# shionhonda/gae-dgl

Hardware: AMD Instinct MI355X
Metric: edges aggregated/sec (SpMM fwd+bwd) (higher is better)
Workload: dtype f32 (storage, aggregations, accumulators; the dense products run on the 16-bit matrix pipe from split operands with fp32 accumulation: X W^T and dW from three bf16 pieces per operand / six pairs, the loss from two fp16 pieces (N >= 5120) or three bf16 pieces -- all fp32-grade, see ms_per_step_exact_

## Files before the change

gae_dgl_amd/csrc/decoder_bce.hip:

```cpp
#include <string.h>

#include "common.h"
#include "bce_finalize.h"

namespace {

using gae::kWave;
typedef float f32x4 __attribute__((ext_vector_type(4)));
typedef short s16x4 __attribute__((ext_vector_type(4)));
typedef float f32x2 __attribute__((ext_vector_type(2)));
typedef __bf16 bf16x2 __attribute__((ext_vector_type(2)));

constexpr int TJ = 64;
constexpr int PREP_ROWS = 64;
constexpr int kBceRi = 2;
constexpr int64_t kBceGrid = 2048;
constexpr int64_t kBceSymGrid = 16384;
constexpr int kChipCus = 256;
}

namespace gae {
Knob g_bce_s_bf16{3};
Knob g_bce_last_kind{0};
Knob g_bce_sym_bal{1};
// ... 499 lines not shown
    }
#pragma unroll
    for (int off = 32; off > 0; off >>= 1) { la += __shfl_down(la, off, 64); ll += __shfl_down(ll, off, 64); }
    if (lane == 0) { red[wave][0] = la; red[wave][1] = ll; }
    __syncthreads();
    if (tid == 0) {
        const int64_t b = int64_t(blockIdx.y) * n_row_blocks + blockIdx.x;
        loss_partial[2 * b + 0] = (red[0][0] + red[1][0]) + (red[2][0] + red[3][0]);
        loss_partial[2 * b + 1] = (red[0][1] + red[1][1]) + (red[2][1] + red[3][1]);
    }
}

}

namespace gae {
Knob g_bce_sym_ri{0};
}

namespace {
using gae::g_bce_sym_ri;

__device__ __forceinline__ s16x4 upper_halves(const f32x4 &d)
{
    struct U { unsigned a, b; } u{__builtin_amdgcn_perm(__float_as_uint(d[1]), __float_as_uint(d[0]), 0x07060302u),
                                  __builtin_amdgcn_perm(__float_as_uint(d[3]), __float_as_uint(d[2]), 0x07060302u)};
    return __builtin_bit_cast(s16x4, u);
}

__host__ __device__ inline int64_t sym_strip_offset(int64_t I, int64_t NP, int64_t PR)
{
    return 16 * (I * NP - PR * (I * (I + 1) / 2));
}

enum class SymForm { kF16, kBf16x3, kBf16x3Fallback };

template <bool WITH_GRAD, int RI, SymForm FORM, bool BAL>
__global__ __launch_bounds__(256, (RI == 2 && FORM != SymForm::kBf16x3Fallback) ? 3 : 2) void bce_dense_sym_kernel(
    const float *__restrict__ Zt , const unsigned short *__restrict__ Zhi,
    const unsigned short *__restrict__ Zlo, int64_t n, int64_t cols_per_chunk,
    float *__restrict__ O_partial , float *__restrict__ Wmir,
    double *__restrict__ loss_partial , const double *__restrict__ colsum_partial,
    int64_t n_prep_blocks, double *__restrict__ S, float *__restrict__ S_all_f, unsigned n_panels, int exp_strip,
    unsigned *__restrict__ range_flag, int flag_mode, unsigned ticket, unsigned n_chunks, int bal_tpb)
{
    if (flag_mode == 2 && *range_flag != ticket) return;
    constexpr bool F16 = FORM == SymForm::kF16;
    constexpr bool PERSIST = FORM == SymForm::kBf16x3Fallback;
    bool out_of_range = false;
    constexpr int DP = 16, SYM_PR = 64 * RI;
    constexpr int LDH = DP + 4;
    constexpr int V4 = TJ * DP / 4 / 256;
    constexpr int LDM = TJ + 4;
    constexpr int LDHL = 2 * DP + 8;
    __shared__ __attribute__((aligned(16))) unsigned short HLs[2][TJ * LDHL];
    __shared__ __attribute__((aligned(16))) unsigned short L2s[2][F16 ? 4 : TJ * LDH];
    __shared__ __attribute__((aligned(16))) float MR[2][4][16 * LDM];
    __shared__ double red[4][2];

  double sumA = 0.0, sumL = 0.0;
  auto unit = [&](const int64_t I, const int64_t col_begin, const int64_t col_end, const int64_t op_slot, const int64_t lp_index) {
    const int tid = threadIdx.x, lane = tid & 63, wave = tid >> 6;
    const int l15 = lane & 15, g = lane >> 4;
    const int64_t NP = (n + 63) / 64 * 64;
    const int64_t row_base = SYM_PR * I + wave * (RI * 16);
    const int64_t diag_end = SYM_PR * (I + 1);

    constexpr float LOG2E = 1.44269504088896341f;
    static_assert(RI % 2 == 0, "row subtiles are paired into K = 32 mirror products");
    s16x8 bhh[RI];
    s16x8 bll[RI];
    s16x8 b3[F16 ? 1 : RI];
    s16x8 zTh[RI / 2], zTl[RI / 2];
#pragma unroll
    for (int ri = 0; ri < RI; ++ri) {
        const int64_t i = row_base + ri * 16 + l15;
        f32x4 b = *reinterpret_cast<const f32x4 *>(Zt + (i < n ? i : 0) * DP + 4 * g);
// ... 254 lines not shown
            if (I > T - 1) I = T - 1;
            I = __builtin_amdgcn_readfirstlane(I);
            while (I > 0 && prefix(I) > t0) --I;
            while (I + 1 < T && prefix(I + 1) <= t0) ++I;
            while (t0 < t1) {
                const int pI = prefix(I), tiles = NT - TPP * I;
                const int lt = t0 - pI;
                int cnt = tiles - lt;
                if (cnt > t1 - t0) cnt = t1 - t0;
                const int64_t cb = int64_t(SYM_PR) * I + int64_t(lt) * 64;
                int64_t ce = cb + int64_t(cnt) * 64;
                if (ce > n) ce = n;
                if (cb < n) unit(I, cb, ce, int(vb) - int(unsigned(pI) / unsigned(bal_tpb)), -1);
                __syncthreads();
                t0 += cnt; ++I;
            }
        }
        const int tid = threadIdx.x, lane = tid & 63, wave = tid >> 6;
        double la = sumA * 0.69314718055994531, ll = sumL;
#pragma unroll
        for (int off = 32; off > 0; off >>= 1) { la += __shfl_down(la, off, 64); ll += __shfl_down(ll, off, 64); }
        if (lane == 0) { red[wave][0] = la; red[wave][1] = ll; }
        __syncthreads();
        if (tid == 0) {
            loss_partial[2 * vb + 0] = (red[0][0] + red[1][0]) + (red[2][0] + red[3][0]);
            loss_partial[2 * vb + 1] = (red[0][1] + red[1][1]) + (red[2][1] + red[3][1]);
        }
        };
        if constexpr (PERSIST) {
            for (unsigned vb = blockIdx.x; vb < n_vb; vb += gridDim.x) {
                vblock(vb);
                __syncthreads();
            }
        } else {
            vblock(blockIdx.x);
        }
    } else if constexpr (PERSIST) {
        const unsigned nx = n_panels + 1, total = nx * n_chunks;
        for (unsigned u = blockIdx.x; u < total; u += gridDim.x) {
            unit_xy(u % nx, u / nx);
            __syncthreads();
        }
    } else {
        unit_xy(blockIdx.x, blockIdx.y);
    }
}

__global__ __launch_bounds__(256) void bce_mirror_reduce_kernel(const float *__restrict__ Wmir, int64_t n,
                                                               float *__restrict__ Omir , int SYM_PR)
{
    const int64_t NP = (n + 63) / 64 * 64;
    const int64_t j0 = int64_t(blockIdx.x) * TJ;
    const int f = threadIdx.x >> 4, jq = (threadIdx.x & 15) * 4;
    const int64_t n_left = j0 / SYM_PR;
    f32x4 acc = {0.f, 0.f, 0.f, 0.f};
    auto at = [&](int64_t I) {
        const int64_t de = SYM_PR * (I + 1);
        return *reinterpret_cast<const f32x4 *>(Wmir + sym_strip_offset(I, NP, SYM_PR) + (j0 - de) * 16 + f * TJ + jq);
    };
    int64_t I = 0;
    for (; I + 8 <= n_left; I += 8) {
        f32x4 v[8];
#pragma unroll
        for (int u = 0; u < 8; ++u) v[u] = at(I + u);
#pragma unroll
        for (int u = 0; u < 8; ++u) acc += v[u];
    }
    for (; I < n_left; ++I) acc += at(I);
#pragma unroll
    for (int e = 0; e < 4; ++e)
        if (j0 + jq + e < n) Omir[(j0 + jq + e) * 16 + f] = acc[e];
}

template <int LPR, bool WITH_GRAD>
__global__ __launch_bounds__(256) void bce_edges_kernel(
    const float *__restrict__ Zt , const float *__restrict__ mask, int64_t ldz,
    int64_t row_begin, int64_t n_local, int d, const int32_t *__restrict__ indptr,
    const int32_t *__restrict__ indices, const int32_t *__restrict__ t_indptr, const int32_t *__restrict__ t_indices,
    float pw, float inv_n2, const float *__restrict__ O_partial, int n_splits, int DP,
    const float *__restrict__ S_all_f, float *__restrict__ dZ, int64_t lddz, double *__restrict__ loss_partial,
    const float *__restrict__ O_mirror , int64_t sym_cols_per_chunk, int SYM_PR,
    const int64_t *__restrict__ counts, const double *__restrict__ scal,
    const float *__restrict__ Wmir ,
    unsigned *__restrict__ range_flag )
{
    constexpr int VEC = 4;
    if (range_flag != nullptr && blockIdx.x == 0 && threadIdx.x == 0) *range_flag = 0u;
    const unsigned bid = (LPR == 4 && Wmir != nullptr) ? gridDim.x - 1u - blockIdx.x : blockIdx.x;
    __shared__ __attribute__((aligned(16))) float Om[LPR == 4 ? TJ * 20 : 4];
    const bool fold = LPR == 4 && Wmir != nullptr;
    if (LPR == 4 && fold) {
        const int64_t NP = (n_local + 63) / 64 * 64;
        const int64_t j0 = int64_t(bid) * TJ;
        const int f = threadIdx.x >> 4, jq = (threadIdx.x & 15) * 4;
        const int64_t n_left = j0 / SYM_PR;
        f32x4 acc = {0.f, 0.f, 0.f, 0.f};
        auto at = [&](int64_t I) {
            const int64_t de = SYM_PR * (I + 1);
            return *reinterpret_cast<const f32x4 *>(Wmir + sym_strip_offset(I, NP, SYM_PR) + (j0 - de) * 16 + f * TJ + jq);
        };
        int64_t I = 0;
        for (; I + 8 <= n_left; I += 8) {
            f32x4 v[8];
#pragma unroll
            for (int u = 0; u < 8; ++u) v[u] = at(I + u);
#pragma unroll
            for (int u = 0; u < 8; ++u) acc += v[u];
        }
        for (; I < n_left; ++I) acc += at(I);
#pragma unroll
        for (int e = 0; e < 4; ++e) Om[(jq + e) * 20 + f] = acc[e];
        __syncthreads();
    }
    if (scal) { pw = float(scal[0]); inv_n2 = float(scal[1]); }
    const int64_t n_valid = counts ? counts[0] : n_local;
    __shared__ double red[4];
    constexpr int RPB = 256 / LPR;
    const int tid = threadIdx.x, lane = tid & 63, wave = tid >> 6;
    const int lig = tid % LPR;
    const int64_t i = int64_t(bid) * RPB + tid / LPR;
    const int64_t gi = row_begin + i;
    const int64_t n = n_local;
    const int f0 = lig * VEC;
    const bool rowv = i < n;
    const bool fv = f0 < DP;

    float zi[VEC], acc_in[VEC], acc_out[VEC];
    const f32x4 zero4 = {0.f, 0.f, 0.f, 0.f};
    {
        const f32x4 t = (rowv && fv) ? *reinterpret_cast<const f32x4 *>(Zt + gi * DP + f0) : zero4;
#pragma unroll
        for (int q = 0; q < VEC; ++q) { acc_in[q] = acc_out[q] = 0.f; zi[q] = t[q]; }
    }
    float sall[VEC], mk[VEC];
#pragma unroll
    for (int q = 0; q < VEC; ++q) {
        const bool in = WITH_GRAD && rowv && f0 + q < d;
        sall[q] = WITH_GRAD ? S_all_f[in ? f0 + q : 0] : 0.f;
        mk[q] = (WITH_GRAD && mask != nullptr) ? mask[in ? gi * ldz + f0 + q : 0] : 1.f;
    }
    int32_t posA = rowv ? indptr[i] : 0;
    int32_t endA = rowv ? indptr[i + 1] : 0;
    int32_t posB = (WITH_GRAD && rowv) ? t_indptr[i] : 0;
    int32_t endB = (WITH_GRAD && rowv) ? t_indptr[i + 1] : 0;
    constexpr int kLongRow = 16;
    const bool is_long = max(endA - posA, endB - posB) > kLongRow;
    const int32_t longA0 = posA, longA1 = endA, longB0 = posB, longB1 = endB;
    if (is_long) { endA = posA; endB = posB; }
    f32x4 osum = zero4;
    if (WITH_GRAD && rowv && fv) {
        const float *op = O_partial + i * DP + f0;
        const int64_t sstride = n * DP;
        if (O_mirror) {
            if (sym_cols_per_chunk < 0) {
                const int64_t tpb = -sym_cols_per_chunk, I = i / SYM_PR, TPP = SYM_PR / 64, NT = (n + 63) / 64;
                const int64_t pI = I * NT - TPP * (I * (I - 1) / 2), pI1 = pI + NT - TPP * I;
                n_splits = int((pI1 - 1) / tpb - pI / tpb + 1);
            } else {
                const int64_t rem = n - (i / SYM_PR) * SYM_PR;
                n_splits = int((rem + sym_cols_per_chunk - 1) / sym_cols_per_chunk);
            }
            osum = fold ? *reinterpret_cast<const f32x4 *>(&Om[(tid / LPR) * 20 + f0])
                        : *reinterpret_cast<const f32x4 *>(O_mirror + i * DP + f0);
        }
        int sp = 0;
        for (; sp + 8 <= n_splits; sp += 8) {
            f32x4 o[8];
#pragma unroll
            for (int u = 0; u < 8; ++u) o[u] = *reinterpret_cast<const f32x4 *>(op + (sp + u) * sstride);
#pragma unroll
            for (int u = 0; u < 8; ++u) osum += o[u];
        }
        if (sp < n_splits) {
            f32x4 o[8];
#pragma unroll
            for (int u = 0; u < 8; ++u) {
                const int su = sp + u < n_splits ? sp + u : n_splits - 1;
                o[u] = *reinterpret_cast<const f32x4 *>(op + su * sstride);
            }
#pragma unroll
            for (int u = 0; u < 8; ++u) osum += (sp + u < n_splits) ? o[u] : zero4;
        }
    }
    double lsum = 0.0;
    constexpr int NE = LPR >= 4 ? 8 : 4;
    const int glane0 = (lane / LPR) * LPR;
    while (posA < endA || posB < endB) {
        int32_t mineA[NE / 4], mineB[NE / 4];
#pragma unroll
        for (int h = 0; h < NE / 4; ++h) {
            const int32_t eA = posA + 4 * h + (LPR >= 4 ? (lig & 3) : 0), eB = posB + 4 * h + (LPR >= 4 ? (lig & 3) : 0);
            mineA[h] = eA < endA ? indices[eA] : 0;
            mineB[h] = (WITH_GRAD && eB < endB) ? t_indices[eB] : 0;
        }
        float zj[2 * NE][VEC], dot[2 * NE];
#pragma unroll
        for (int u = 0; u < 2 * NE; ++u) {
            const bool second = u >= NE;
            if (second && !WITH_GRAD) { dot[u] = 0.f; continue; }
            const int32_t pos = second ? posB : posA, end = second ? endB : endA;
            const int uu = u % NE;
            const int32_t mine = second ? mineB[uu / 4] : mineA[uu / 4];
            const int32_t j = LPR >= 4 ? __shfl(mine, glane0 + (uu & 3), 64)
                                       : (pos + uu < end ? (second ? t_indices : indices)[pos + uu] : 0);
            const bool ev = pos + uu < end;
            dot[u] = 0.f;
            const f32x4 t = (ev && fv) ? *reinterpret_cast<const f32x4 *>(Zt + int64_t(j) * DP + f0) : zero4;
#pragma unroll
            for (int q = 0; q < VEC; ++q) {
                zj[u][q] = t[q];
                dot[u] = fmaf(zi[q], t[q], dot[u]);
            }
        }
#pragma unroll
        for (int off = LPR / 2; off > 0; off >>= 1)
#pragma unroll
            for (int u = 0; u < (WITH_GRAD ? 2 * NE : NE); ++u) dot[u] += __shfl_xor(dot[u], off, 64);
#pragma unroll
        for (int u = 0; u < (WITH_GRAD ? 2 * NE : NE); ++u) {
            const bool second = u >= NE;
            const int32_t pos = second ? posB : posA, end = second ? endB : endA;
            if (pos + (u % NE) < end) {
                const float x = dot[u];
                float spn, sgn;
                softplus_sigmoid(-x, spn, sgn);
                const float sg = 1.0f - sgn;
                if (!second && lig == 0) lsum += double(-x + (pw - 1.0f) * spn);
                const float c = (pw - 1.0f) * sg - pw;
#pragma unroll
                for (int q = 0; q < VEC; ++q) {
                    if (second) acc_out[q] = fmaf(c, zj[u][q], acc_out[q]);
                    else acc_in[q] = fmaf(c, zj[u][q], acc_in[q]);
                }
            }
        }
        posA = min(posA + NE, endA);
        posB = min(posB + NE, endB);
    }
    {
        constexpr int G = 64 / LPR, CU = LPR < 4 ? LPR : 4, CH = CU * G;
        unsigned long long todo = __builtin_amdgcn_ballot_w64(is_long && lig == 0);
        const int grp = lane / LPR;
        while (todo != 0) {
            const int hl = __builtin_ctzll(todo);
            todo &= todo - 1;
            const int32_t eA = __builtin_amdgcn_readlane(longA1, hl), eB = __builtin_amdgcn_readlane(longB1, hl);
            int32_t a0 = __builtin_amdgcn_readlane(longA0, hl), b0 = __builtin_amdgcn_readlane(longB0, hl);
            float zr[VEC], pin[VEC], pout[VEC];
#pragma unroll
            for (int q = 0; q < VEC; ++q) {
                zr[q] = __shfl(zi[q], hl + lig, 64);
                pin[q] = pout[q] = 0.f;
            }
            for (; a0 < eA || b0 < eB; a0 += CH, b0 += CH) {
                const int32_t idA = (lane < CH && a0 + lane < eA) ? indices[a0 + lane] : 0;
                const int32_t idB = (WITH_GRAD && lane < CH && b0 + lane < eB) ? t_indices[b0 + lane] : 0;
                float zj[2 * CU][VEC], dot[2 * CU];
#pragma unroll
                for (int u = 0; u < 2 * CU; ++u) {
                    const bool second = u >= CU;
                    dot[u] = 0.f;
                    if (second && !WITH_GRAD) continue;
                    const int slot = grp + G * (u % CU);
                    const int32_t j = __shfl(second ? idB : idA, slot, 64);
                    const bool ev = (second ? b0 : a0) + slot < (second ? eB : eA);
                    const f32x4 t = (ev && fv) ? *reinterpret_cast<const f32x4 *>(Zt + int64_t(j) * DP + f0) : zero4;
#pragma unroll
                    for (int q = 0; q < VEC; ++q) {
                        zj[u][q] = t[q];
                        dot[u] = fmaf(zr[q], t[q], dot[u]);
                    }
                }
#pragma unroll
                for (int off = LPR / 2; off > 0; off >>= 1)
#pragma unroll
                    for (int u = 0; u < (WITH_GRAD ? 2 * CU : CU); ++u) dot[u] += __shfl_xor(dot[u], off, 64);
#pragma unroll
                for (int u = 0; u < (WITH_GRAD ? 2 * CU : CU); ++u) {
                    const bool second = u >= CU;
                    const int slot = grp + G * (u % CU);
                    if ((second ? b0 : a0) + slot < (second ? eB : eA)) {
                        const float x = dot[u];
                        float spn, sgn;
                        softplus_sigmoid(-x, spn, sgn);
                        const float sg = 1.0f - sgn;
                        if (!second && lig == 0) lsum += double(-x + (pw - 1.0f) * spn);
                        const float c = (pw - 1.0f) * sg - pw;
#pragma unroll
                        for (int q = 0; q < VEC; ++q) {
                            if (second) pout[q] = fmaf(c, zj[u][q], pout[q]);
                            else pin[q] = fmaf(c, zj[u][q], pin[q]);
                        }
                    }
                }
            }
#pragma unroll
            for (int off = LPR; off < 64; off <<= 1)
#pragma unroll
                for (int q = 0; q < VEC; ++q) {
                    pin[q] += __shfl_xor(pin[q], off, 64);
                    if (WITH_GRAD) pout[q] += __shfl_xor(pout[q], off, 64);
                }
            if ((lane & ~(LPR - 1)) == hl) {
#pragma unroll
                for (int q = 0; q < VEC; ++q) { acc_in[q] += pin[q]; acc_out[q] += pout[q]; }
            }
        }
    }
    if (WITH_GRAD && rowv) {
#pragma unroll
        for (int q = 0; q < VEC; ++q) {
            const int f = f0 + q;
            if (f < d) {
                const float o = 0.5f * sall[q] + osum[q];
                float v = (2.0f * o + (acc_in[q] + acc_out[q])) * inv_n2;
                if (mask) v *= mk[q];
                if (i >= n_valid) v = 0.f;
                dZ[i * lddz + f] = v;
            }
        }
    }
#pragma unroll
    for (int off = 32; off > 0; off >>= 1) lsum += __shfl_down(lsum, off, 64);
    if (lane == 0) red[wave] = lsum;
    __syncthreads();
    if (tid == 0) loss_partial[bid] = (red[0] + red[1]) + (red[2] + red[3]);
}

__global__ __launch_bounds__(1024) void bce_finalize_kernel(const gae_bce_tail t)
{
    __shared__ double red[3][16];
    gae::bce_finalize_block<1024>(t, red);
}

struct BcePlan {
    int64_t row_blocks, n_splits, cols_per_split, edge_blocks, prep_blocks;
    int KS, DP, LPR;
    int64_t o_bytes, zt_bytes, zh_bytes, cs_bytes, s_bytes, n_dense, total_bytes;
    double pad_terms;
    bool sym;
    int sym_pr;
    int bal_tpb;
    int64_t bal_blocks;
    int64_t wmir_bytes, omir_bytes;
};

inline int64_t align256(int64_t x) { return (x + 255) / 256 * 256; }

bool bce_plan(int64_t n, int64_t n_local, int64_t d, BcePlan &p)
{
    const int64_t ROWS_PER_BLOCK = 64 * kBceRi;
    if (d > 64) return false;
    p.KS = int((d + 15) / 16);
    if (p.KS == 3) p.KS = 4;
    if (p.KS < 1) p.KS = 1;
    p.DP = p.KS * 16;
    p.row_blocks = (n_local + ROWS_PER_BLOCK - 1) / ROWS_PER_BLOCK;
    if (p.row_blocks < 1) p.row_blocks = 1;
    int64_t col_tiles = (n + TJ - 1) / TJ;
    if (col_tiles < 1) col_tiles = 1;
    int64_t want = (kBceGrid + p.row_blocks - 1) / p.row_blocks;
    if (want > col_tiles) want = col_tiles;
    if (want > 32) want = 32;
    if (want < 1) want = 1;
    const int64_t tiles_per_split = (col_tiles + want - 1) / want;
    p.cols_per_split = tiles_per_split * TJ;
    p.n_splits = (col_tiles + tiles_per_split - 1) / tiles_per_split;
    p.pad_terms = double(col_tiles * TJ - n) * double(n_local);
    const int nvec = p.DP / 4;
    int lpr = 1;
    while (lpr < nvec) lpr <<= 1;
    p.LPR = lpr;
    p.edge_blocks = (n_local + (256 / lpr) - 1) / (256 / lpr);
    if (p.edge_blocks < 1) p.edge_blocks = 1;
    p.prep_blocks = (n + PREP_ROWS - 1) / PREP_ROWS;
    p.sym = false;
    p.sym_pr = 128;
    p.bal_tpb = 0;
    p.bal_blocks = 0;
    p.wmir_bytes = p.omir_bytes = 0;
    const bool bal = g_bce_sym_bal == 2 || (g_bce_sym_bal == 1 && n < 65536);
    if (g_bce_sym && n_local == n && p.KS == 1 && g_bce_s_bf16 && g_bce_pv_bf16 &&
        n >= (g_bce_sym > 1 ? 512 : (bal ? 5120 : 8192))) {
        const int64_t SYM_PR = (g_bce_sym_ri == 4 || (g_bce_sym_ri == 0 && (n >= 32768 || bal))) ? 256 : 128;
        p.sym_pr = int(SYM_PR);
        const int64_t T = (n + SYM_PR - 1) / SYM_PR, NP = (n + 63) / 64 * 64;
        int64_t chunks = (kBceSymGrid + T - 1) / T;
        if (chunks > 28) chunks = 28;
        if (chunks > col_tiles) chunks = col_tiles;
        if (chunks < 1) chunks = 1;
        int64_t cpc = ((n + chunks - 1) / chunks + TJ - 1) / TJ * TJ;
        const int64_t slots = int64_t(kChipCus) * (SYM_PR == 128 ? 3 : 2);
        auto live_blocks = [&](int64_t t) {
            int64_t L = 0;
            for (int64_t I = 0; I < T; ++I) L += (n - SYM_PR * I + t * TJ - 1) / (t * TJ);
            return L;
        };
        const int64_t t0 = cpc / TJ;
        if ((live_blocks(t0) + slots - 1) / slots <= 6) {
            double best = -1.0;
            int64_t best_t = t0;
            for (int64_t t = t0 - t0 / 4; t <= t0 + t0 / 4; ++t) {
                if (t < 1) continue;
                const int64_t L = live_blocks(t), rounds = (L + slots - 1) / slots;
                const double fill = double(L) / double(rounds * slots) - 0.002 * double(t > t0 ? t - t0 : t0 - t);
                if (fill > best) { best = fill; best_t = t; }
            }
            cpc = best_t * TJ;
        }
        const int64_t last_len = NP - SYM_PR * T;
        const int64_t wfloats = sym_strip_offset(T - 1, NP, SYM_PR) + 16 * (last_len > 0 ? last_len : 0);
        if (wfloats * 4 <= (int64_t(8) << 30)) {
            p.sym = true;
            p.row_blocks = T;
            p.cols_per_split = cpc;
            p.n_splits = (n + cpc - 1) / cpc;
            p.pad_terms = 0.0;
            p.wmir_bytes = align256(wfloats * 4);
            p.omir_bytes = align256(n * 16 * 4);
            if (bal) {
                const int64_t TPP = SYM_PR / TJ, NT = NP / TJ;
                auto prefix = [&](int64_t I) { return I * NT - TPP * (I * (I - 1) / 2); };
                const int64_t W = prefix(T), slots = int64_t(kChipCus) * (SYM_PR == 128 ? 3 : 2);
                const int64_t tpb = (W + slots - 1) / slots;
                int64_t most = 1;
                for (int64_t I = 0; I < T; ++I) {
                    const int64_t pieces = (prefix(I + 1) - 1) / tpb - prefix(I) / tpb + 1;
                    if (pieces > most) most = pieces;
                }
                p.bal_tpb = int(tpb);
                p.bal_blocks = (W + tpb - 1) / tpb;
                p.n_splits = most;
            }
        }
    }
    p.o_bytes = align256(p.n_splits * n_local * p.DP * 4);
    p.zt_bytes = align256(n * p.DP * 4);
    p.zh_bytes = align256(n * p.DP * 2);
    p.cs_bytes = align256(((n + 15) / 16 + 1) * 2 * p.DP * 8);
    p.s_bytes = align256(2 * p.DP * 8 + p.DP * 4 + 4 * 8);
    p.n_dense = p.bal_tpb ? p.bal_blocks : p.row_blocks * p.n_splits;
    p.total_bytes = p.o_bytes + p.zt_bytes + 2 * p.zh_bytes + p.cs_bytes + p.s_bytes +
                    align256((2 * p.n_dense + p.edge_blocks) * 8) + p.wmir_bytes + p.omir_bytes;
    return true;
}

template <int KS, bool WITH_GRAD>
auto dense_kernel()
{
    if (!g_bce_s_bf16) return bce_dense_kernel<KS, WITH_GRAD, false, false>;
    return g_bce_pv_bf16 ? bce_dense_kernel<KS, WITH_GRAD, true, true> : bce_dense_kernel<KS, WITH_GRAD, true, false>;
}

template <bool WITH_GRAD>
int launch_dense(const BcePlan &p, const float *Zt, const unsigned short *Zhi, const unsigned short *Zlo, int64_t n,
                 int64_t row_begin, int64_t n_local, float *O, double *lp, const double *cs, double *S, float *S_all_f,
                 hipStream_t s)
{
    const dim3 grid(unsigned(p.row_blocks) + 1, unsigned(p.n_splits));
    const auto kernel = p.KS == 1 ? dense_kernel<1, WITH_GRAD>() : p.KS == 2 ? dense_kernel<2, WITH_GRAD>()
                                                                             : dense_kernel<4, WITH_GRAD>();
    hipLaunchKernelGGL(kernel, grid, dim3(256), 0, s, Zt, Zhi, Zlo, n, row_begin, n_local, p.cols_per_split, O, lp, cs,
                       p.prep_blocks, S, S_all_f, unsigned(p.row_blocks));
    GAE_CHECK_LAUNCH("bce_dense_kernel");
    return GAE_OK;
}

template <bool WITH_GRAD>
int launch_edges(const BcePlan &p, const float *Zt, const float *mask, int64_t ldz, int64_t row_begin, int64_t n, int d,
                 const int32_t *ip, const int32_t *ix, const int32_t *tp, const int32_t *tx, float pw, float inv_n2,
                 const float *O, const float *S_all_f, float *dZ, int64_t lddz, double *lp, const float *Omir,
                 const int64_t *counts, const double *scal, const float *Wmir, unsigned *range_flag, hipStream_t s)
{
    const auto kernel = p.LPR == 1 ? bce_edges_kernel<1, WITH_GRAD>
                        : p.LPR == 2 ? bce_edges_kernel<2, WITH_GRAD>
                        : p.LPR == 4 ? bce_edges_kernel<4, WITH_GRAD>
                        : p.LPR == 8 ? bce_edges_kernel<8, WITH_GRAD>
                                     : bce_edges_kernel<16, WITH_GRAD>;
    hipLaunchKernelGGL(kernel, dim3(unsigned(p.edge_blocks)), dim3(256), 0, s, Zt, mask, ldz, row_begin, n, d, ip, ix, tp,
                       tx, pw, inv_n2, O, int(p.n_splits), p.DP, S_all_f, dZ, lddz, lp, Omir,
                       (p.bal_tpb ? -int64_t(p.bal_tpb) : p.cols_per_split), p.sym_pr, counts, scal, Wmir, range_flag);
    GAE_CHECK_LAUNCH("bce_edges_kernel");
    return GAE_OK;
}

template <SymForm FORM>
auto sym_kernel(const BcePlan &p, bool with_grad)
{
    const bool tall = p.sym_pr == 256, bal = p.bal_tpb != 0;
    if (with_grad) {
        if (tall) return bal ? bce_dense_sym_kernel<true, 4, FORM, true> : bce_dense_sym_kernel<true, 4, FORM, false>;
        return bal ? bce_dense_sym_kernel<true, 2, FORM, true> : bce_dense_sym_kernel<true, 2, FORM, false>;
    }
    if (tall) return bal ? bce_dense_sym_kernel<false, 4, FORM, true> : bce_dense_sym_kernel<false, 4, FORM, false>;
    return bal ? bce_dense_sym_kernel<false, 2, FORM, true> : bce_dense_sym_kernel<false, 2, FORM, false>;
}

}

extern "C" int64_t gae_decoder_bce_workspace_bytes(int64_t n, int64_t n_local, int64_t d)
{
    if (n < 0 || d < 0 || n_local < 0 || n_local > n) return GAE_E_SIZE;
    BcePlan p;
    if (!bce_plan(n, n_local, d, p)) return GAE_E_RANGE;
    return p.total_bytes + 256;
}

namespace {
inline double bce_all_pairs(const BcePlan &p, int64_t n, int64_t n_local)
{
    return p.sym ? double(n) * double(n) : double(n_local) * double((n + TJ - 1) / TJ * TJ);
}

thread_local gae_bce_tail *t_tail_out = nullptr;
// ... 12 lines not shown
    GAE_REQUIRE(n > 0 && d > 0, GAE_E_SIZE, "gae_decoder_bce: n and d must be positive");
    GAE_REQUIRE(row_begin >= 0 && n_local >= 0 && row_begin + n_local <= n, GAE_E_SIZE,
                "gae_decoder_bce: row window outside [0, n)");
    GAE_REQUIRE(d <= 64, GAE_E_RANGE, "gae_decoder_bce: d = %lld > 64 not supported by the fused kernel",
                (long long)d);
    GAE_REQUIRE(n < (int64_t(1) << 31), GAE_E_SIZE, "gae_decoder_bce: n too large");
    GAE_REQUIRE(ldz >= d && (!dZ || lddz >= d), GAE_E_SIZE, "gae_decoder_bce: leading dimension too small");
    GAE_REQUIRE((Z || prepared) && loss_out && workspace && (n_local == 0 || indptr), GAE_E_NULL, "gae_decoder_bce: NULL pointer");
    GAE_REQUIRE(!dZ || n_local == 0 || t_indptr, GAE_E_NULL, "gae_decoder_bce: the gradient needs the CSR of A^T");
    BcePlan p;
    bce_plan(n, n_local, d, p);
    GAE_REQUIRE(workspace_bytes >= p.total_bytes, GAE_E_WORKSPACE, "gae_decoder_bce: workspace %lld < %lld bytes",
                (long long)workspace_bytes, (long long)p.total_bytes);
    if (prepared) {
        GAE_REQUIRE(prepared_blocks >= 1 && prepared_blocks * 2 * p.DP * 8 <= p.cs_bytes, GAE_E_RANGE,
                    "gae_x_decoder_bce_prepared: %lld column-sum partials do not fit the workspace", (long long)prepared_blocks);
        p.prep_blocks = prepared_blocks;
    }
    GAE_REQUIRE(gae::aligned16(workspace), GAE_E_ALIGN, "gae_decoder_bce: workspace not 16-byte aligned");
    hipStream_t s = gae::as_stream(stream);
    char *w = static_cast<char *>(workspace);
    float *O = reinterpret_cast<float *>(w); w += p.o_bytes;
    float *Zt = reinterpret_cast<float *>(w); w += p.zt_bytes;
    unsigned short *Zhi = reinterpret_cast<unsigned short *>(w); w += p.zh_bytes;
    unsigned short *Zlo = reinterpret_cast<unsigned short *>(w); w += p.zh_bytes;
    double *cs = reinterpret_cast<double *>(w); w += p.cs_bytes;
    double *S = reinterpret_cast<double *>(w);
    float *S_all_f = reinterpret_cast<float *>(w + 2 * p.DP * 8);
    double *scal = counts ? reinterpret_cast<double *>(w + 2 * p.DP * 8 + ((p.DP * 4 + 7) & ~7)) : nullptr;
    unsigned *range_flag = reinterpret_cast<unsigned *>(w + 2 * p.DP * 8 + ((p.DP * 4 + 7) & ~7) + 3 * 8);
    w += p.s_bytes;
    double *lp = reinterpret_cast<double *>(w); w += align256((2 * p.n_dense + p.edge_blocks) * 8);
    float *Wmir = reinterpret_cast<float *>(w); w += p.wmir_bytes;
    float *Omir = reinterpret_cast<float *>(w);
    const double inv_n2 = 1.0 / (double(n) * double(n));
    if (n_local == 0) {
        GAE_HIP(hipMemsetAsync(loss_out, 0, sizeof(float), s));
        if (t_tail_out) { memset(t_tail_out, 0, sizeof(gae_bce_tail)); t_tail_out = nullptr; }
        return GAE_OK;
    }
    if (!prepared) {
        hipLaunchKernelGGL(bce_prepare_kernel, dim3(unsigned(p.prep_blocks)), dim3(256), 0, s, Z, mask, ldz, n, int(d), p.DP,
                           row_begin, row_begin + n_local, Zt, Zhi, Zlo, cs, dropout_p, 1.0f / (1.0f - dropout_p), seed,
                           offset, draw_dev, counts, scal, bce_all_pairs(p, n, n_local));
        GAE_CHECK_LAUNCH("bce_prepare_kernel");
    }
    int rc;
    g_bce_last_kind = p.sym ? (p.sym_pr == 256 ? 3 : 2) : 1;
    if (p.sym) {
        const dim3 grid = p.bal_tpb ? dim3(unsigned(p.bal_blocks) + 1) : dim3(unsigned(p.row_blocks) + 1, unsigned(p.n_splits));
        static std::atomic<unsigned> call_counter{0};
        const unsigned ticket = (call_counter.fetch_add(1) * 2654435761u) | 0x80000001u;
        auto launch_sym = [&](auto kernel, dim3 g, int flag_mode) {
            hipLaunchKernelGGL(kernel, g, dim3(256), 0, s, Zt, Zhi, Zlo, n, p.cols_per_split, O, Wmir, lp, cs, p.prep_blocks, S,
                               S_all_f, unsigned(p.row_blocks), n >= 32768 ? 1 : 0, range_flag, flag_mode, ticket,
                               (p.bal_tpb ? unsigned(p.bal_blocks) + 1u : unsigned(p.n_splits)), p.bal_tpb);
        };
        if (g_bce_s_bf16 == 3) {
            launch_sym(sym_kernel<SymForm::kF16>(p, dZ != nullptr), grid, 1);
            launch_sym(sym_kernel<SymForm::kBf16x3Fallback>(p, dZ != nullptr), p.bal_tpb ? dim3(64) : dim3(2 * kChipCus), 2);
        } else {
            launch_sym(sym_kernel<SymForm::kBf16x3>(p, dZ != nullptr), grid, 0);
        }
        GAE_CHECK_LAUNCH("bce_dense_sym_kernel");
        if (dZ && p.LPR != 4) {
            hipLaunchKernelGGL(bce_mirror_reduce_kernel, dim3(unsigned((n + TJ - 1) / TJ)), dim3(256), 0, s, Wmir, n,
                               Omir, p.sym_pr);
            GAE_CHECK_LAUNCH("bce_mirror_reduce_kernel");
        }
        rc = GAE_OK;
    } else {
        rc = dZ ? launch_dense<true>(p, Zt, Zhi, Zlo, n, row_begin, n_local, O, lp, cs, S, S_all_f, s)
                : launch_dense<false>(p, Zt, Zhi, Zlo, n, row_begin, n_local, O, lp, cs, S, S_all_f, s);
    }
    if (rc) return rc;
    double *lpe = lp + 2 * p.n_dense;
    rc = dZ ? launch_edges<true>(p, Zt, mask, ldz, row_begin, n_local, int(d), indptr, indices, t_indptr, t_indices,
                                    pos_weight, float(inv_n2), O, S_all_f, dZ, lddz, lpe, p.sym ? Omir : nullptr,
                                    counts, scal, (p.sym && p.LPR == 4) ? Wmir : nullptr,
                                    p.sym ? range_flag : nullptr, s)
            : launch_edges<false>(p, Zt, mask, ldz, row_begin, n_local, int(d), indptr, indices, t_indptr,
                                     t_indices, pos_weight, float(inv_n2), O, S_all_f, dZ, lddz, lpe, nullptr, counts,
                                     scal, nullptr, p.sym ? range_flag : nullptr, s);
    if (rc) return rc;
    gae_bce_tail tail;
    memset(&tail, 0, sizeof(tail));
    tail.dense_partial = lp; tail.n_dense = p.n_dense;
    tail.edge_partial = lpe; tail.n_edge = p.edge_blocks;
    tail.S = S; tail.DP = p.DP;
    tail.pad_terms = p.pad_terms; tail.inv_n2 = inv_n2;
    tail.loss_out = loss_out; tail.bump_draw = dropout_p > 0.f ? draw_dev : nullptr; tail.scal = scal;
    if (t_tail_out) {
        *t_tail_out = tail;
        t_tail_out = nullptr;
        return GAE_OK;
    }
    hipLaunchKernelGGL(bce_finalize_kernel, dim3(1), dim3(1024), 0, s, tail);
    GAE_CHECK_LAUNCH("bce_finalize_kernel");
    return GAE_OK;
}
}

extern "C" int gae_x_decoder_bce_defer_finalize(gae_bce_tail *tail_out)
{
    t_tail_out = tail_out;
    return GAE_OK;
}

extern "C" int gae_x_decoder_bce_finalize(const gae_bce_tail *tail, void *stream)
{
    GAE_REQUIRE(tail != nullptr, GAE_E_NULL, "gae_x_decoder_bce_finalize: tail is NULL");
    if (tail->loss_out == nullptr) return GAE_OK;
    GAE_REQUIRE(tail->S && (tail->n_dense == 0 || tail->dense_partial) && (tail->n_edge == 0 || tail->edge_partial) &&
                    tail->DP > 0 && tail->n_dense >= 0 && tail->n_edge >= 0,
                GAE_E_NULL, "gae_x_decoder_bce_finalize: malformed tail (not one written by gae_decoder_bce*)");
    hipLaunchKernelGGL(bce_finalize_kernel, dim3(1), dim3(1024), 0, gae::as_stream(stream), *tail);
// ... 72 lines not shown
```

Before: 1.319 billion.

## Run sparse edge walk inside balanced symmetric dense kernel as extra blocks

Moves the per-row sparse edge walk (dot products, softplus/sigmoid, gradient accumulation over positive edges) into extra blocks appended to the balanced symmetric dense BCE launch. The walk's partial gradient goes to a scratch buffer, and the edges kernel becomes a lighter combine pass that only adds the dense and mirror terms. The aim is to overlap the latency-bound gather walk with the matrix-core dense work and shorten the serial edges kernel. The cost is a larger grid for the dense kernel, an extra n×16 float scratch buffer, and possible contention with the dense blocks for CU slots.

New measurement: 1.345 billion, median of 6. 1.02x the previous value.

```diff
diff --git a/gae_dgl_amd/csrc/decoder_bce.hip b/gae_dgl_amd/csrc/decoder_bce.hip
--- a/gae_dgl_amd/csrc/decoder_bce.hip
+++ b/gae_dgl_amd/csrc/decoder_bce.hip
@@ -555,6 +555,199 @@
     return 16 * (I * NP - PR * (I * (I + 1) / 2));
 }
 
+template <int LPR, bool WITH_GRAD>
+struct EdgeWalk {
+    static constexpr int VEC = 4;
+    static constexpr int kLongRow = 16;
+    float zi[VEC], acc_in[VEC], acc_out[VEC];
+    int32_t posA, endA, posB, endB, longA0, longA1, longB0, longB1;
+    bool is_long;
+
+    __device__ __forceinline__ void start(const float *__restrict__ Zt, int DP, int64_t i, int64_t gi, bool rowv,
+                                          int f0, bool fv, const int32_t *__restrict__ indptr,
+                                          const int32_t *__restrict__ t_indptr)
+    {
+        const f32x4 zero4 = {0.f, 0.f, 0.f, 0.f};
+        const f32x4 t = (rowv && fv) ? *reinterpret_cast<const f32x4 *>(Zt + gi * DP + f0) : zero4;
+#pragma unroll
+        for (int q = 0; q < VEC; ++q) { acc_in[q] = acc_out[q] = 0.f; zi[q] = t[q]; }
+        posA = rowv ? indptr[i] : 0;
+        endA = rowv ? indptr[i + 1] : 0;
+        posB = (WITH_GRAD && rowv) ? t_indptr[i] : 0;
+        endB = (WITH_GRAD && rowv) ? t_indptr[i + 1] : 0;
+        is_long = max(endA - posA, endB - posB) > kLongRow;
+        longA0 = posA; longA1 = endA; longB0 = posB; longB1 = endB;
+        if (is_long) { endA = posA; endB = posB; }
+    }
+
+    __device__ __forceinline__ double run(const float *__restrict__ Zt, int DP, int f0, bool fv, float pw,
+                                          const int32_t *__restrict__ indices, const int32_t *__restrict__ t_indices)
+    {
+        const f32x4 zero4 = {0.f, 0.f, 0.f, 0.f};
+        const int lane = threadIdx.x & 63, lig = threadIdx.x % LPR;
+        double lsum = 0.0;
+        constexpr int NE = LPR >= 4 ? 8 : 4;
+        const int glane0 = (lane / LPR) * LPR;
+        while (posA < endA || posB < endB) {
+            int32_t mineA[NE / 4], mineB[NE / 4];
+#pragma unroll
+            for (int h = 0; h < NE / 4; ++h) {
+                const int32_t eA = posA + 4 * h + (LPR >= 4 ? (lig & 3) : 0), eB = posB + 4 * h + (LPR >= 4 ? (lig & 3) : 0);
+                mineA[h] = eA < endA ? indices[eA] : 0;
+                mineB[h] = (WITH_GRAD && eB < endB) ? t_indices[eB] : 0;
+            }
+            float zj[2 * NE][VEC], dot[2 * NE];
+#pragma unroll
+            for (int u = 0; u < 2 * NE; ++u) {
+                const bool second = u >= NE;
+                if (second && !WITH_GRAD) { dot[u] = 0.f; continue; }
+                const int32_t pos = second ? posB : posA, end = second ? endB : endA;
+                const int uu = u % NE;
+                const int32_t mine = second ? mineB[uu / 4] : mineA[uu / 4];
+                const int32_t j = LPR >= 4 ? __shfl(mine, glane0 + (uu & 3), 64)
+                                           : (pos + uu < end ? (second ? t_indices : indices)[pos + uu] : 0);
+                const bool ev = pos + uu < end;
+                dot[u] = 0.f;
+                const f32x4 t = (ev && fv) ? *reinterpret_cast<const f32x4 *>(Zt + int64_t(j) * DP + f0) : zero4;
+#pragma unroll
+                for (int q = 0; q < VEC; ++q) {
+                    zj[u][q] = t[q];
+                    dot[u] = fmaf(zi[q], t[q], dot[u]);
+                }
+            }
+#pragma unroll
+            for (int off = LPR / 2; off > 0; off >>= 1)
+#pragma unroll
+                for (int u = 0; u < (WITH_GRAD ? 2 * NE : NE); ++u) dot[u] += __shfl_xor(dot[u], off, 64);
+#pragma unroll
+            for (int u = 0; u < (WITH_GRAD ? 2 * NE : NE); ++u) {
+                const bool second = u >= NE;
+                const int32_t pos = second ? posB : posA, end = second ? endB : endA;
+                if (pos + (u % NE) < end) {
+                    const float x = dot[u];
+                    float spn, sgn;
+                    softplus_sigmoid(-x, spn, sgn);
+                    const float sg = 1.0f - sgn;
+                    if (!second && lig == 0) lsum += double(-x + (pw - 1.0f) * spn);
+                    const float c = (pw - 1.0f) * sg - pw;
+#pragma unroll
+                    for (int q = 0; q < VEC; ++q) {
+                        if (second) acc_out[q] = fmaf(c, zj[u][q], acc_out[q]);
+                        else acc_in[q] = fmaf(c, zj[u][q], acc_in[q]);
+                    }
+                }
+            }
+            posA = min(posA + NE, endA);
+            posB = min(posB + NE, endB);
+        }
+        {
+            constexpr int G = 64 / LPR, CU = LPR < 4 ? LPR : 4, CH = CU * G;
+            unsigned long long todo = __builtin_amdgcn_ballot_w64(is_long && lig == 0);
+            const int grp = lane / LPR;
+            while (todo != 0) {
+                const int hl = __builtin_ctzll(todo);
+                todo &= todo - 1;
+                const int32_t eA = __builtin_amdgcn_readlane(longA1, hl), eB = __builtin_amdgcn_readlane(longB1, hl);
+                int32_t a0 = __builtin_amdgcn_readlane(longA0, hl), b0 = __builtin_amdgcn_readlane(longB0, hl);
+                float zr[VEC], pin[VEC], pout[VEC];
+#pragma unroll
+                for (int q = 0; q < VEC; ++q) {
+                    zr[q] = __shfl(zi[q], hl + lig, 64);
+                    pin[q] = pout[q] = 0.f;
+                }
+                for (; a0 < eA || b0 < eB; a0 += CH, b0 += CH) {
+                    const int32_t idA = (lane < CH && a0 + lane < eA) ? indices[a0 + lane] : 0;
+                    const int32_t idB = (WITH_GRAD && lane < CH && b0 + lane < eB) ? t_indices[b0 + lane] : 0;
+                    float zj[2 * CU][VEC], dot[2 * CU];
+#pragma unroll
+                    for (int u = 0; u < 2 * CU; ++u) {
+                        const bool second = u >= CU;
+                        dot[u] = 0.f;
+                        if (second && !WITH_GRAD) continue;
+                        const int slot = grp + G * (u % CU);
+                        const int32_t j = __shfl(second ? idB : idA, slot, 64);
+                        const bool ev = (second ? b0 : a0) + slot < (second ? eB : eA);
+                        const f32x4 t = (ev && fv) ? *reinterpret_cast<const f32x4 *>(Zt + int64_t(j) * DP + f0) : zero4;
+#pragma unroll
+                        for (int q = 0; q < VEC; ++q) {
+                            zj[u][q] = t[q];
+                            dot[u] = fmaf(zr[q], t[q], dot[u]);
+                        }
+                    }
+#pragma unroll
+                    for (int off = LPR / 2; off > 0; off >>= 1)
+#pragma unroll
+                        for (int u = 0; u < (WITH_GRAD ? 2 * CU : CU); ++u) dot[u] += __shfl_xor(dot[u], off, 64);
+#pragma unroll
+                    for (int u = 0; u < (WITH_GRAD ? 2 * CU : CU); ++u) {
+                        const bool second = u >= CU;
+                        const int slot = grp + G * (u % CU);
+                        if ((second ? b0 : a0) + slot < (second ? eB : eA)) {
+                            const float x = dot[u];
+                            float spn, sgn;
+                            softplus_sigmoid(-x, spn, sgn);
+                            const float sg = 1.0f - sgn;
+                            if (!second && lig == 0) lsum += double(-x + (pw - 1.0f) * spn);
+                            const float c = (pw - 1.0f) * sg - pw;
+#pragma unroll
+                            for (int q = 0; q < VEC; ++q) {
+                                if (second) pout[q] = fmaf(c, zj[u][q], pout[q]);
+                                else pin[q] = fmaf(c, zj[u][q], pin[q]);
+                            }
+                        }
+                    }
+                }
+#pragma unroll
+                for (int off = LPR; off < 64; off <<= 1)
+#pragma unroll
+                    for (int q = 0; q < VEC; ++q) {
+                        pin[q] += __shfl_xor(pin[q], off, 64);
+                        if (WITH_GRAD) pout[q] += __shfl_xor(pout[q], off, 64);
+                    }
+                if ((lane & ~(LPR - 1)) == hl) {
+#pragma unroll
+                    for (int q = 0; q < VEC; ++q) { acc_in[q] += pin[q]; acc_out[q] += pout[q]; }
+                }
+            }
+        }
+        return lsum;
+    }
+};
+
+struct SymWalkArgs {
+    const int32_t *indptr, *indices, *t_indptr, *t_indices;
+    float pw;
+    const double *scal;
+    float *s;
+    double *loss_partial;
+    unsigned n_walk;
+};
+
+__device__ __forceinline__ void sym_walk_block(const float *__restrict__ Zt, int64_t n, unsigned w, const SymWalkArgs &wk,
+                                               double (*red)[2])
+{
+    constexpr int LPR = 4, DP = 16;
+    const int tid = threadIdx.x, lane = tid & 63, wave = tid >> 6;
+    const int64_t i = int64_t(w) * (256 / LPR) + tid / LPR;
+    const bool rowv = i < n;
+    const int f0 = (tid % LPR) * 4;
+    const float pw = wk.scal ? float(wk.scal[0]) : wk.pw;
+    EdgeWalk<LPR, true> ew;
+    ew.start(Zt, DP, i, i, rowv, f0, true, wk.indptr, wk.t_indptr);
+    double lsum = ew.run(Zt, DP, f0, true, pw, wk.indices, wk.t_indices);
+    if (rowv) {
+        f32x4 v;
+#pragma unroll
+        for (int q = 0; q < 4; ++q) v[q] = ew.acc_in[q] + ew.acc_out[q];
+        *reinterpret_cast<f32x4 *>(wk.s + i * DP + f0) = v;
+    }
+#pragma unroll
+    for (int off = 32; off > 0; off >>= 1) lsum += __shfl_down(lsum, off, 64);
+    if (lane == 0) red[wave][0] = lsum;
+    __syncthreads();
+    if (tid == 0) wk.loss_partial[w] = (red[0][0] + red[1][0]) + (red[2][0] + red[3][0]);
+}
+
 enum class SymForm { kF16, kBf16x3, kBf16x3Fallback };
 
 template <bool WITH_GRAD, int RI, SymForm FORM, bool BAL>
@@ -564,7 +757,8 @@
     float *__restrict__ O_partial , float *__restrict__ Wmir,
     double *__restrict__ loss_partial , const double *__restrict__ colsum_partial,
     int64_t n_prep_blocks, double *__restrict__ S, float *__restrict__ S_all_f, unsigned n_panels, int exp_strip,
-    unsigned *__restrict__ range_flag, int flag_mode, unsigned ticket, unsigned n_chunks, int bal_tpb)
+    unsigned *__restrict__ range_flag, int flag_mode, unsigned ticket, unsigned n_chunks, int bal_tpb,
+    const SymWalkArgs wk)
 {
     if (flag_mode == 2 && *range_flag != ticket) return;
     constexpr bool F16 = FORM == SymForm::kF16;
@@ -885,6 +1079,9 @@
                 vblock(vb);
                 __syncthreads();
             }
+        } else if (WITH_GRAD && blockIdx.x >= n_vb) {
+            const unsigned w = blockIdx.x - n_vb;
+            if (w < wk.n_walk) sym_walk_block(Zt, n, w, wk, red);
         } else {
             vblock(blockIdx.x);
         }
@@ -925,7 +1122,7 @@
         if (j0 + jq + e < n) Omir[(j0 + jq + e) * 16 + f] = acc[e];
 }
 
-template <int LPR, bool WITH_GRAD>
+template <int LPR, bool WITH_GRAD, bool WALK = true>
 __global__ __launch_bounds__(256) void bce_edges_kernel(
     const float *__restrict__ Zt , const float *__restrict__ mask, int64_t ldz,
     int64_t row_begin, int64_t n_local, int d, const int32_t *__restrict__ indptr,
@@ -935,9 +1132,11 @@
     const float *__restrict__ O_mirror , int64_t sym_cols_per_chunk, int SYM_PR,
     const int64_t *__restrict__ counts, const double *__restrict__ scal,
     const float *__restrict__ Wmir ,
-    unsigned *__restrict__ range_flag )
-{
-    constexpr int VEC = 4;
+    unsigned *__restrict__ range_flag ,
+    const float *__restrict__ s_walk )
+{
+    static_assert(WALK || (LPR == 4 && WITH_GRAD), "the combine follows the walk blocks of the balanced symmetric launch");
+    constexpr int VEC = EdgeWalk<LPR, WITH_GRAD>::VEC;
     if (range_flag != nullptr && blockIdx.x == 0 && threadIdx.x == 0) *range_flag = 0u;
     const unsigned bid = (LPR == 4 && Wmir != nullptr) ? gridDim.x - 1u - blockIdx.x : blockIdx.x;
     __shared__ __attribute__((aligned(16))) float Om[LPR == 4 ? TJ * 20 : 4];
@@ -978,13 +1177,11 @@
     const bool rowv = i < n;
     const bool fv = f0 < DP;
 
-    float zi[VEC], acc_in[VEC], acc_out[VEC];
+    EdgeWalk<LPR, WITH_GRAD> ew;
     const f32x4 zero4 = {0.f, 0.f, 0.f, 0.f};
-    {
-        const f32x4 t = (rowv && fv) ? *reinterpret_cast<const f32x4 *>(Zt + gi * DP + f0) : zero4;
-#pragma unroll
-        for (int q = 0; q < VEC; ++q) { acc_in[q] = acc_out[q] = 0.f; zi[q] = t[q]; }
-    }
+    f32x4 sw = zero4;
+    if constexpr (WALK) ew.start(Zt, DP, i, gi, rowv, f0, fv, indptr, t_indptr);
+    else if (rowv) sw = *reinterpret_cast<const f32x4 *>(s_walk + i * 16 + f0);
     float sall[VEC], mk[VEC];
 #pragma unroll
     for (int q = 0; q < VEC; ++q) {
@@ -992,14 +1189,6 @@
         sall[q] = WITH_GRAD ? S_all_f[in ? f0 + q : 0] : 0.f;
         mk[q] = (WITH_GRAD && mask != nullptr) ? mask[in ? gi * ldz + f0 + q : 0] : 1.f;
     }
-    int32_t posA = rowv ? indptr[i] : 0;
-    int32_t endA = rowv ? indptr[i + 1] : 0;
-    int32_t posB = (WITH_GRAD && rowv) ? t_indptr[i] : 0;
-    int32_t endB = (WITH_GRAD && rowv) ? t_indptr[i + 1] : 0;
-    constexpr int kLongRow = 16;
-    const bool is_long = max(endA - posA, endB - posB) > kLongRow;
-    const int32_t longA0 = posA, longA1 = endA, longB0 = posB, longB1 = endB;
-    if (is_long) { endA = posA; endB = posB; }
     f32x4 osum = zero4;
     if (WITH_GRAD && rowv && fv) {
         const float *op = O_partial + i * DP + f0;
@@ -1036,143 +1225,22 @@
         }
     }
     double lsum = 0.0;
-    constexpr int NE = LPR >= 4 ? 8 : 4;
-    const int glane0 = (lane / LPR) * LPR;
-    while (posA < endA || posB < endB) {
-        int32_t mineA[NE / 4], mineB[NE / 4];
-#pragma unroll
-        for (int h = 0; h < NE / 4; ++h) {
-            const int32_t eA = posA + 4 * h + (LPR >= 4 ? (lig & 3) : 0), eB = posB + 4 * h + (LPR >= 4 ? (lig & 3) : 0);
-            mineA[h] = eA < endA ? indices[eA] : 0;
-            mineB[h] = (WITH_GRAD && eB < endB) ? t_indices[eB] : 0;
-        }
-        float zj[2 * NE][VEC], dot[2 * NE];
-#pragma unroll
-        for (int u = 0; u < 2 * NE; ++u) {
-            const bool second = u >= NE;
-            if (second && !WITH_GRAD) { dot[u] = 0.f; continue; }
-            const int32_t pos = second ? posB : posA, end = second ? endB : endA;
-            const int uu = u % NE;
-            const int32_t mine = second ? mineB[uu / 4] : mineA[uu / 4];
-            const int32_t j = LPR >= 4 ? __shfl(mine, glane0 + (uu & 3), 64)
-                                       : (pos + uu < end ? (second ? t_indices : indices)[pos + uu] : 0);
-            const bool ev = pos + uu < end;
-            dot[u] = 0.f;
-            const f32x4 t = (ev && fv) ? *reinterpret_cast<const f32x4 *>(Zt + int64_t(j) * DP + f0) : zero4;
-#pragma unroll
-            for (int q = 0; q < VEC; ++q) {
-                zj[u][q] = t[q];
-                dot[u] = fmaf(zi[q], t[q], dot[u]);
-            }
-        }
-#pragma unroll
-        for (int off = LPR / 2; off > 0; off >>= 1)
-#pragma unroll
-            for (int u = 0; u < (WITH_GRAD ? 2 * NE : NE); ++u) dot[u] += __shfl_xor(dot[u], off, 64);
-#pragma unroll
-        for (int u = 0; u < (WITH_GRAD ? 2 * NE : NE); ++u) {
-            const bool second = u >= NE;
-            const int32_t pos = second ? posB : posA, end = second ? endB : endA;
-            if (pos + (u % NE) < end) {
-                const float x = dot[u];
-                float spn, sgn;
-                softplus_sigmoid(-x, spn, sgn);
-                const float sg = 1.0f - sgn;
-                if (!second && lig == 0) lsum += double(-x + (pw - 1.0f) * spn);
-                const float c = (pw - 1.0f) * sg - pw;
-#pragma unroll
-                for (int q = 0; q < VEC; ++q) {
-                    if (second) acc_out[q] = fmaf(c, zj[u][q], acc_out[q]);
-                    else acc_in[q] = fmaf(c, zj[u][q], acc_in[q]);
-                }
-            }
-        }
-        posA = min(posA + NE, endA);
-        posB = min(posB + NE, endB);
-    }
-    {
-        constexpr int G = 64 / LPR, CU = LPR < 4 ? LPR : 4, CH = CU * G;
-        unsigned long long todo = __builtin_amdgcn_ballot_w64(is_long && lig == 0);
-        const int grp = lane / LPR;
-        while (todo != 0) {
-            const int hl = __builtin_ctzll(todo);
-            todo &= todo - 1;
-            const int32_t eA = __builtin_amdgcn_readlane(longA1, hl), eB = __builtin_amdgcn_readlane(longB1, hl);
-            int32_t a0 = __builtin_amdgcn_readlane(longA0, hl), b0 = __builtin_amdgcn_readlane(longB0, hl);
-            float zr[VEC], pin[VEC], pout[VEC];
-#pragma unroll
-            for (int q = 0; q < VEC; ++q) {
-                zr[q] = __shfl(zi[q], hl + lig, 64);
-                pin[q] = pout[q] = 0.f;
-            }
-            for (; a0 < eA || b0 < eB; a0 += CH, b0 += CH) {
-                const int32_t idA = (lane < CH && a0 + lane < eA) ? indices[a0 + lane] : 0;
-                const int32_t idB = (WITH_GRAD && lane < CH && b0 + lane < eB) ? t_indices[b0 + lane] : 0;
-                float zj[2 * CU][VEC], dot[2 * CU];
-#pragma unroll
-                for (int u = 0; u < 2 * CU; ++u) {
-                    const bool second = u >= CU;
-                    dot[u] = 0.f;
-                    if (second && !WITH_GRAD) continue;
-                    const int slot = grp + G * (u % CU);
-                    const int32_t j = __shfl(second ? idB : idA, slot, 64);
-                    const bool ev = (second ? b0 : a0) + slot < (second ? eB : eA);
-                    const f32x4 t = (ev && fv) ? *reinterpret_cast<const f32x4 *>(Zt + int64_t(j) * DP + f0) : zero4;
-#pragma unroll
-                    for (int q = 0; q < VEC; ++q) {
-                        zj[u][q] = t[q];
-                        dot[u] = fmaf(zr[q], t[q], dot[u]);
-                    }
-                }
-#pragma unroll
-                for (int off = LPR / 2; off > 0; off >>= 1)
-#pragma unroll
-                    for (int u = 0; u < (WITH_GRAD ? 2 * CU : CU); ++u) dot[u] += __shfl_xor(dot[u], off, 64);
-#pragma unroll
-                for (int u = 0; u < (WITH_GRAD ? 2 * CU : CU); ++u) {
-                    const bool second = u >= CU;
-                    const int slot = grp + G * (u % CU);
-                    if ((second ? b0 : a0) + slot < (second ? eB : eA)) {
-                        const float x = dot[u];
-                        float spn, sgn;
-                        softplus_sigmoid(-x, spn, sgn);
-                        const float sg = 1.0f - sgn;
-                        if (!second && lig == 0) lsum += double(-x + (pw - 1.0f) * spn);
-                        const float c = (pw - 1.0f) * sg - pw;
-#pragma unroll
-                        for (int q = 0; q < VEC; ++q) {
-                            if (second) pout[q] = fmaf(c, zj[u][q], pout[q]);
-                            else pin[q] = fmaf(c, zj[u][q], pin[q]);
-                        }
-                    }
-                }
-            }
-#pragma unroll
-            for (int off = LPR; off < 64; off <<= 1)
-#pragma unroll
-                for (int q = 0; q < VEC; ++q) {
-                    pin[q] += __shfl_xor(pin[q], off, 64);
-                    if (WITH_GRAD) pout[q] += __shfl_xor(pout[q], off, 64);
-                }
-            if ((lane & ~(LPR - 1)) == hl) {
-#pragma unroll
-                for (int q = 0; q < VEC; ++q) { acc_in[q] += pin[q]; acc_out[q] += pout[q]; }
-            }
-        }
-    }
+    if constexpr (WALK) lsum = ew.run(Zt, DP, f0, fv, pw, indices, t_indices);
     if (WITH_GRAD && rowv) {
 #pragma unroll
         for (int q = 0; q < VEC; ++q) {
             const int f = f0 + q;
             if (f < d) {
                 const float o = 0.5f * sall[q] + osum[q];
-                float v = (2.0f * o + (acc_in[q] + acc_out[q])) * inv_n2;
+                const float sparse = WALK ? ew.acc_in[q] + ew.acc_out[q] : sw[q];
+                float v = (2.0f * o + sparse) * inv_n2;
                 if (mask) v *= mk[q];
                 if (i >= n_valid) v = 0.f;
                 dZ[i * lddz + f] = v;
             }
         }
     }
+    if constexpr (!WALK) return;
 #pragma unroll
     for (int off = 32; off > 0; off >>= 1) lsum += __shfl_down(lsum, off, 64);
     if (lane == 0) red[wave] = lsum;
@@ -1196,6 +1264,7 @@
     int bal_tpb;
     int64_t bal_blocks;
     int64_t wmir_bytes, omir_bytes;
+    int64_t sw_bytes;
 };
 
 inline int64_t align256(int64_t x) { return (x + 255) / 256 * 256; }
@@ -1232,6 +1301,7 @@
     p.bal_tpb = 0;
     p.bal_blocks = 0;
     p.wmir_bytes = p.omir_bytes = 0;
+    p.sw_bytes = 0;
     const bool bal = g_bce_sym_bal == 2 || (g_bce_sym_bal == 1 && n < 65536);
     if (g_bce_sym && n_local == n && p.KS == 1 && g_bce_s_bf16 && g_bce_pv_bf16 &&
         n >= (g_bce_sym > 1 ? 512 : (bal ? 5120 : 8192))) {
@@ -1284,6 +1354,7 @@
                 p.bal_tpb = int(tpb);
                 p.bal_blocks = (W + tpb - 1) / tpb;
                 p.n_splits = most;
+                p.sw_bytes = align256(n * 16 * 4);
             }
         }
     }
@@ -1294,7 +1365,7 @@
     p.s_bytes = align256(2 * p.DP * 8 + p.DP * 4 + 4 * 8);
     p.n_dense = p.bal_tpb ? p.bal_blocks : p.row_blocks * p.n_splits;
     p.total_bytes = p.o_bytes + p.zt_bytes + 2 * p.zh_bytes + p.cs_bytes + p.s_bytes +
-                    align256((2 * p.n_dense + p.edge_blocks) * 8) + p.wmir_bytes + p.omir_bytes;
+                    align256((2 * p.n_dense + p.edge_blocks) * 8) + p.wmir_bytes + p.omir_bytes + p.sw_bytes;
     return true;
 }
 
@@ -1323,8 +1394,16 @@
 int launch_edges(const BcePlan &p, const float *Zt, const float *mask, int64_t ldz, int64_t row_begin, int64_t n, int d,
                  const int32_t *ip, const int32_t *ix, const int32_t *tp, const int32_t *tx, float pw, float inv_n2,
                  const float *O, const float *S_all_f, float *dZ, int64_t lddz, double *lp, const float *Omir,
-                 const int64_t *counts, const double *scal, const float *Wmir, unsigned *range_flag, hipStream_t s)
-{
+                 const int64_t *counts, const double *scal, const float *Wmir, unsigned *range_flag,
+                 const float *s_walk , hipStream_t s)
+{
+    if (WITH_GRAD && s_walk) {
+        hipLaunchKernelGGL((bce_edges_kernel<4, true, false>), dim3(unsigned(p.edge_blocks)), dim3(256), 0, s, Zt, mask,
+                           ldz, row_begin, n, d, ip, ix, tp, tx, pw, inv_n2, O, int(p.n_splits), p.DP, S_all_f, dZ, lddz,
+                           lp, Omir, -int64_t(p.bal_tpb), p.sym_pr, counts, scal, Wmir, range_flag, s_walk);
+        GAE_CHECK_LAUNCH("bce_edges_kernel (combine)");
+        return GAE_OK;
+    }
     const auto kernel = p.LPR == 1 ? bce_edges_kernel<1, WITH_GRAD>
                         : p.LPR == 2 ? bce_edges_kernel<2, WITH_GRAD>
                         : p.LPR == 4 ? bce_edges_kernel<4, WITH_GRAD>
@@ -1332,7 +1411,8 @@
                                      : bce_edges_kernel<16, WITH_GRAD>;
     hipLaunchKernelGGL(kernel, dim3(unsigned(p.edge_blocks)), dim3(256), 0, s, Zt, mask, ldz, row_begin, n, d, ip, ix, tp,
                        tx, pw, inv_n2, O, int(p.n_splits), p.DP, S_all_f, dZ, lddz, lp, Omir,
-                       (p.bal_tpb ? -int64_t(p.bal_tpb) : p.cols_per_split), p.sym_pr, counts, scal, Wmir, range_flag);
+                       (p.bal_tpb ? -int64_t(p.bal_tpb) : p.cols_per_split), p.sym_pr, counts, scal, Wmir, range_flag,
+                       nullptr);
     GAE_CHECK_LAUNCH("bce_edges_kernel");
     return GAE_OK;
 }
@@ -1411,7 +1491,8 @@
     w += p.s_bytes;
     double *lp = reinterpret_cast<double *>(w); w += align256((2 * p.n_dense + p.edge_blocks) * 8);
     float *Wmir = reinterpret_cast<float *>(w); w += p.wmir_bytes;
-    float *Omir = reinterpret_cast<float *>(w);
+    float *Omir = reinterpret_cast<float *>(w); w += p.omir_bytes;
+    float *s_walk = reinterpret_cast<float *>(w);
     const double inv_n2 = 1.0 / (double(n) * double(n));
     if (n_local == 0) {
         GAE_HIP(hipMemsetAsync(loss_out, 0, sizeof(float), s));
@@ -1425,15 +1506,20 @@
         GAE_CHECK_LAUNCH("bce_prepare_kernel");
     }
     int rc;
+    double *lpe = lp + 2 * p.n_dense;
+    const bool walk_in_dense = p.sym && p.bal_tpb && p.LPR == 4 && dZ != nullptr;
     g_bce_last_kind = p.sym ? (p.sym_pr == 256 ? 3 : 2) : 1;
     if (p.sym) {
-        const dim3 grid = p.bal_tpb ? dim3(unsigned(p.bal_blocks) + 1) : dim3(unsigned(p.row_blocks) + 1, unsigned(p.n_splits));
+        SymWalkArgs wk{indptr, indices, t_indptr, t_indices, pos_weight, scal, s_walk, lpe,
+                       walk_in_dense ? unsigned(p.edge_blocks) : 0u};
+        const dim3 grid = p.bal_tpb ? dim3(unsigned(p.bal_blocks) + 1 + wk.n_walk)
+                                    : dim3(unsigned(p.row_blocks) + 1, unsigned(p.n_splits));
         static std::atomic<unsigned> call_counter{0};
         const unsigned ticket = (call_counter.fetch_add(1) * 2654435761u) | 0x80000001u;
         auto launch_sym = [&](auto kernel, dim3 g, int flag_mode) {
             hipLaunchKernelGGL(kernel, g, dim3(256), 0, s, Zt, Zhi, Zlo, n, p.cols_per_split, O, Wmir, lp, cs, p.prep_blocks, S,
                                S_all_f, unsigned(p.row_blocks), n >= 32768 ? 1 : 0, range_flag, flag_mode, ticket,
-                               (p.bal_tpb ? unsigned(p.bal_blocks) + 1u : unsigned(p.n_splits)), p.bal_tpb);
+                               (p.bal_tpb ? unsigned(p.bal_blocks) + 1u : unsigned(p.n_splits)), p.bal_tpb, wk);
         };
         if (g_bce_s_bf16 == 3) {
             launch_sym(sym_kernel<SymForm::kF16>(p, dZ != nullptr), grid, 1);
@@ -1453,14 +1539,13 @@
                 : launch_dense<false>(p, Zt, Zhi, Zlo, n, row_begin, n_local, O, lp, cs, S, S_all_f, s);
     }
     if (rc) return rc;
-    double *lpe = lp + 2 * p.n_dense;
     rc = dZ ? launch_edges<true>(p, Zt, mask, ldz, row_begin, n_local, int(d), indptr, indices, t_indptr, t_indices,
                                     pos_weight, float(inv_n2), O, S_all_f, dZ, lddz, lpe, p.sym ? Omir : nullptr,
                                     counts, scal, (p.sym && p.LPR == 4) ? Wmir : nullptr,
-                                    p.sym ? range_flag : nullptr, s)
+                                    p.sym ? range_flag : nullptr, walk_in_dense ? s_walk : nullptr, s)
             : launch_edges<false>(p, Zt, mask, ldz, row_begin, n_local, int(d), indptr, indices, t_indptr,
                                      t_indices, pos_weight, float(inv_n2), O, S_all_f, dZ, lddz, lpe, nullptr, counts,
-                                     scal, nullptr, p.sym ? range_flag : nullptr, s);
+                                     scal, nullptr, p.sym ? range_flag : nullptr, nullptr, s);
     if (rc) return rc;
     gae_bce_tail tail;
     memset(&tail, 0, sizeof(tail));
```
